# sandyz1000/face-landmark-detector

Hardware: AMD Instinct MI355X
Metric: faces/sec (whole node), 256x256 batch inference: fused preprocess + FCN-8 forward + softmax + top-4 landmark decode + similarity/alignment warp (higher is better)
Workload: dtype f32; 1 GPU; BASELINE configs[1]: batch=64/GPU 256x256x3 uint8 crops, fcn_8(68) vanilla encoder fp32, random-init weights (seed 2), decode top-4 thresh 0, align to 256x256; global_batch=64, parallelism=dp1

## Files before the change

face-landmark-detector_amd/build.py:

```python
from __future__ import annotations

import concurrent.futures
import hashlib
import os
import shutil
import subprocess
import sys

HERE = os.path.dirname(os.path.abspath(__file__))
ROOT = os.path.dirname(HERE)
CSRC = os.path.join(HERE, "csrc")
INCLUDE = os.path.join(ROOT, "include")
OBJ_DIR = os.path.join(HERE, "csrc", "build")
LIB_PATH = os.path.join(HERE, "libflm_hip.so")

SOURCES = [
    "flm_api.hip",
    "flm_pack.hip",
    "flm_enc1.hip",
    "flm_igemm.hip",
    "flm_igemm_bf16.hip",
    "flm_conv3_halo.hip",
    "flm_score1x1.hip",
    "flm_tail_bf16.hip",
    "flm_convt.hip",
    "flm_up3_wreg.hip",
    "flm_decode.hip",
    "flm_misc.hip",
    "flm_mobile.hip",
]
FLAGS = ["--offload-arch=gfx950", "-O3", "-fPIC", "-std=c++17", "-ffp-contract=off",
         "-Wall", "-Wno-unused-function", "-I", INCLUDE, "-I", CSRC]


FILE_FLAGS = {"flm_enc1.hip": ["-mllvm", "-amdgpu-mfma-vgpr-form"]}


def _hipcc() -> str:
    for c in (shutil.which("hipcc"), "/opt/rocm/bin/hipcc"):
        if c and os.path.exists(c):
            return c
    raise RuntimeError("hipcc not found: the HIP extension cannot be built")


def _stamp(paths) -> str:
    h = hashlib.sha256()
    h.update(" ".join(FLAGS).encode())
    h.update(repr(sorted(FILE_FLAGS.items())).encode())
    for p in sorted(paths):
        with open(p, "rb") as f:
            h.update(p.encode())
            h.update(f.read())
    return h.hexdigest()


def build(force: bool = False, verbose: bool = True, extra_flags=()) -> str:
    os.makedirs(OBJ_DIR, exist_ok=True)
    headers = [os.path.join(CSRC, f) for f in os.listdir(CSRC) if f.endswith(".h")] + \
              [os.path.join(INCLUDE, f) for f in os.listdir(INCLUDE) if f.endswith(".h")]
    srcs = [os.path.join(CSRC, s) for s in SOURCES]
    stamp = _stamp(srcs + headers) + " ".join(extra_flags)
    stamp_file = os.path.join(OBJ_DIR, "stamp.txt")
    if not force and os.path.exists(LIB_PATH) and os.path.exists(stamp_file) and open(stamp_file).read() == stamp:
        return LIB_PATH
    hipcc = _hipcc()

    def compile_one(src):
        obj = os.path.join(OBJ_DIR, os.path.basename(src) + ".o")
        cmd = [hipcc, *FLAGS, *FILE_FLAGS.get(os.path.basename(src), []), *extra_flags, "-c", src, "-o", obj]
        r = subprocess.run(cmd, capture_output=True, text=True)
        if r.returncode != 0:
            raise RuntimeError("hipcc failed on %s:\n%s\n%s" % (src, r.stdout, r.stderr))
        if verbose and r.stderr.strip():
            sys.stderr.write(r.stderr)
        return obj

    with concurrent.futures.ThreadPoolExecutor(max_workers=min(8, len(srcs))) as ex:
        objs = list(ex.map(compile_one, srcs))
    cmd = [hipcc, "--offload-arch=gfx950", "-shared", "-fPIC", "-o", LIB_PATH, *objs]
    r = subprocess.run(cmd, capture_output=True, text=True)
    if r.returncode != 0:
        raise RuntimeError("link failed:\n%s\n%s" % (r.stdout, r.stderr))
    with open(stamp_file, "w") as f:
        f.write(stamp)
    if verbose:
        print("built", LIB_PATH)
    return LIB_PATH


if __name__ == "__main__":
    build(force="--force" in sys.argv)
```

face-landmark-detector_amd/csrc/flm_api.hip:

```cpp
#include <cstdarg>
#include <cstdio>
#include <cstring>

#include "flm_common.h"

namespace flm {

static thread_local char g_err[512] = "";

void set_error(const char* fmt, ...) {
  va_list ap;
  va_start(ap, fmt);
  vsnprintf(g_err, sizeof(g_err), fmt, ap);
  va_end(ap);
}

int hip_fail(hipError_t e, const char* what) {
  set_error("HIP error %d (%s) at %s", (int)e, hipGetErrorString(e), what);
  return FLM_ERR_HIP;
}

struct ProfRec {
  const char* name;
  hipEvent_t a, b;
// ... 35 lines not shown
    return false;
  }
  c->enable = o->landmark_candidates != 0;
  c->sub = o->candidate_sub_phases;
  c->cap_div = o->candidate_cap_div;
  return true;
}
static int cand_sub_for(const CandOpts& c, int n_points, bool bf16) {
  if (c.sub > 0) return c.sub;
  return n_points <= 8 ? (bf16 ? 4 : 2) : (n_points <= 15 ? 6 : 8);
}
static bool landmark_candidates_enabled(const CandOpts& c, const ConvTGeom& g, int fcn32, int decode_mode, int n_points,
                                        int oh, int ow) {
  return c.enable && !fcn32 && decode_mode == FLM_DECODE_TOPN && n_points >= 1 && n_points <= 32 &&
         convt_candidates_supported(g) && (long long)oh * ow < (1 << 17);
}

struct EncNames {
  char s[kMaxEnc][8];
  EncNames() {
    for (int i = 0; i < kMaxEnc; ++i) snprintf(s[i], sizeof(s[i]), "enc%d", i + 1);
  }
};

static size_t take(size_t& cur, size_t bytes) {
  size_t o = cur;
  cur = align_up(cur + bytes, 256);
  return o;
}

Fcn8Ws fcn8_ws_layout(int n, int h, int w, int C, int dtype, int out_mode, int decode_mode, int n_points,
                      int arch, const flm_forward_opts* opts) {
  Fcn8Ws W;
  CandOpts co;
  if (!resolve_opts(opts, &co)) {
    W = Fcn8Ws();
    W.total = 0;
    return W;
  }
  const ConvTGeom g = convt_geom(C, dtype);
  const ArchSpec A = arch_spec(arch);
  const size_t es = dtype == FLM_BF16 ? 2 : 4;
  size_t cur = 0;
  int hs[kMaxEnc], wsz[kMaxEnc];
  enc_dims(A, h, w, hs, wsz);
  for (int i = 0; i < A.n_enc; ++i) W.act[i] = take(cur, es * (size_t)n * hs[i] * wsz[i] * A.enc[i].cout);
  for (int k = 0; k < 5; ++k) W.f[k] = W.act[A.f_idx[k]];
  const int h5 = h / 32, w5 = w / 32, h4 = h / 16, w4 = w / 16, h3 = h / 8, w3 = w / 8;
  W.fc6 = take(cur, es * (size_t)n * h5 * w5 * kFc);
  W.fc7 = take(cur, es * (size_t)n * h5 * w5 * kFc);
  W.score5 = take(cur, sizeof(float) * (size_t)n * h5 * w5 * g.Cp);
  W.fuse4 = take(cur, sizeof(float) * (size_t)n * h4 * w4 * g.Cp);
  W.seg = take(cur, sizeof(float) * (size_t)n * h3 * w3 * g.Cp);
  W.splitk_bytes = sizeof(float) * 8 * (size_t)n * h5 * w5 * g.Cp;
  {
    const size_t rows = (size_t)n * h5 * w5 < 256 ? (size_t)n * h5 * w5 : 256;
    const size_t fc_bytes = sizeof(float) * 8 * rows * kFc;
    if (fc_bytes > W.splitk_bytes) W.splitk_bytes = fc_bytes;
  }
  if (n <= 4) {
    const size_t enc3_bytes = sizeof(float) * 4 * (size_t)4 * (h / 4) * (w / 4) * 256;
    if (enc3_bytes > W.splitk_bytes) W.splitk_bytes = enc3_bytes;
  }
  W.splitk = take(cur, W.splitk_bytes);
  W.oh = h + (A.fcn32 ? 32 : 8);
  W.ow = w + (A.fcn32 ? 32 : 8);
  W.probs = SIZE_MAX;
  W.decode = SIZE_MAX;
  W.sub = W.tau = W.cand = W.cand_cnt = SIZE_MAX;
  W.cand_cap = 0;
  if (out_mode == FLM_OUT_LANDMARKS) {
    W.probs = take(cur, sizeof(float) * (size_t)n * W.oh * W.ow * C);
    W.decode = take(cur, decode_ws_bytes(n, W.oh, W.ow, C, decode_mode, n_points));
    if (landmark_candidates_enabled(co, g, A.fcn32, decode_mode, n_points, W.oh, W.ow)) {
      const int h3 = h / 8, w3 = w / 8;
      W.sub = take(cur, sizeof(unsigned) * (size_t)n * convt_sample_slots(g, h3, w3, cand_sub_for(co, n_points, g.bf16 != 0)) * 16 * g.MT);
      W.tau = take(cur, sizeof(float) * (size_t)n * C);
      W.cand_cap = (int)align_up((size_t)C * 64 * n_points * 4 / co.cap_div, 64);
      if (W.cand_cap < 64) W.cand_cap = 64;
      W.cand = take(cur, sizeof(unsigned long long) * (size_t)n * W.cand_cap);
      W.cand_cnt = take(cur, sizeof(unsigned) * ((size_t)n + 1));
    }
  }
  W.total = cur;
  return W;
}

static int check_fcn8_shape(int n, int h, int w, int C, int dtype) {
  if (dtype != FLM_F32 && dtype != FLM_BF16) {
    set_error("fcn8: unknown dtype %d (FLM_F32 = 0, FLM_BF16 = 1)", dtype);
    return FLM_ERR_UNSUPPORTED;
  }
  if (n <= 0 || h <= 0 || w <= 0 || (h % 32) || (w % 32)) {
    set_error("fcn8: input must be [N>0, H, W, 3] with H and W multiples of 32 (got n=%d h=%d w=%d)", n, h, w);
    return FLM_ERR_SHAPE;
  }
  if (C < 1 || C > kMaxClasses) {
    set_error("fcn8: n_classes must be in [1,%d] (got %d)", kMaxClasses, C);
    return FLM_ERR_SHAPE;
  }
  if (n > (1 << 24) || h > (1 << 15) || w > (1 << 15) || (long long)n * (h + 32) * (w + 32) * C >= (1ll << 40)) {
    set_error("fcn8: batch too large (n=%d h=%d w=%d: at most 2^40 output values per call)", n, h, w);
    return FLM_ERR_SHAPE;
  }
  return FLM_OK;
}

static int conv_layer(hipStream_t s, const char* blob, const ConvPack& c, const void* x, void* y, int n, int h,
                      int w, int relu, int pool, int posmajor, int dtype, int out_f32 = 0,
                      float* splitk_ws = nullptr, size_t splitk_bytes = 0, int stride = 1,
                      const void* res = nullptr) {
  IgemmDesc d;
  d.bf16 = dtype == FLM_BF16;
  d.out_f32 = out_f32;
  d.stride = stride;
  d.res = res;
  d.splitk_ws = splitk_ws;
  d.splitk_ws_bytes = splitk_bytes;
  d.x = x;
  d.wt = blob + c.w;
  d.scale = reinterpret_cast<const float*>(blob + c.scale);
  d.shift = reinterpret_cast<const float*>(blob + c.shift);
  d.y = y;
  d.n = n; d.h = h; d.w = w; d.cin = c.cin;
  d.cout = c.cout; d.coutpad = c.coutpad; d.ldc = c.cout;
  d.kh = c.kh; d.kw = c.kw; d.pad = c.pad;
  d.relu = relu; d.pool = pool; d.posmajor = posmajor;
  return launch_igemm(s, d);
}

}

using namespace flm;

extern "C" {

int flm_abi_version(void) { return FLM_ABI_VERSION; }

int flm_debug_query(const char* key, int arg) {
  if (key && !strcmp(key, "igemm_occupancy")) return igemm_occupancy((size_t)arg);
  return -1;
}

int flm_set_tuning(const char* key, int value) {
  if (!key) return FLM_ERR_ARG;
  if (!strcmp(key, "none")) return FLM_OK;
  if (!strcmp(key, "bf16_big_tiles")) {
    flm::igemm_bf16_big_enable(value);
    return FLM_OK;
  }
  if (!strcmp(key, "f32_two_level")) {
    flm::igemm_f32_group(value ? 0 : -1);
    return FLM_OK;
  }
  if (!strcmp(key, "bf16_mfma16")) {
    flm::igemm_bf16_big_m16(value);
    return FLM_OK;
  }
  if (!strcmp(key, "bf16_halo_mfma16")) {
    flm::conv3_halo_m16(value);
    return FLM_OK;
  }
  if (!strcmp(key, "bf16_lds_dma")) {
    flm::igemm_bf16_big_dma(value);
    return FLM_OK;
  }
  if (!strcmp(key, "landmark_candidates") || !strcmp(key, "candidate_sub_phases") || !strcmp(key, "candidate_cap_div")) {
    set_error("flm_set_tuning: '%s' changes the workspace layout and is a per-call option now: pass flm_forward_opts to "
              "flm_fcn_workspace_bytes_opts / flm_fcn_forward_opts", key);
    return FLM_ERR_ARG;
  }
  if (!strcmp(key, "up3_cand8")) {
    if (value < 0 || value > 7) {
      set_error("flm_set_tuning: up3_cand8 must be in [0,7]");
      return FLM_ERR_ARG;
    }
    flm::convt_cand8_enable(value);
    return FLM_OK;
  }
  if (!strcmp(key, "up3_cand8_rows")) {
    if (value < 0 || value > 8 || (value & (value - 1))) {
      set_error("flm_set_tuning: up3_cand8_rows must be 0, 1, 2, 4 or 8");
      return FLM_ERR_ARG;
    }
    flm::convt_cand8_rows(value);
    return FLM_OK;
  }
  if (!strcmp(key, "up3_wreg")) {
    if (value < 0 || value > 1) {
      set_error("flm_set_tuning: up3_wreg must be 0 or 1");
      return FLM_ERR_ARG;
    }
    flm::convt_wreg_enable(value);
    return FLM_OK;
  }
  if (!strcmp(key, "bf16_score1x1")) {
    flm::score1x1_enable(value);
    return FLM_OK;
  }
  if (!strcmp(key, "bf16_fused_tail")) {
    flm::tail_fused_enable(value);
    return FLM_OK;
  }
  if (!strcmp(key, "decode_lds_dma")) {
    flm::decode_dma_enable(value);
    return FLM_OK;
  }
  if (!strcmp(key, "posmajor_order")) {
    flm::igemm_posperm_enable(value);
    return FLM_OK;
  }
  if (!strcmp(key, "warp_rows")) {
    if (value != 0 && value != 1 && value != 4) {
      set_error("flm_set_tuning: warp_rows must be 0, 1 or 4");
      return FLM_ERR_ARG;
    }
    flm::warp_rows_enable(value);
    return FLM_OK;
  }
  if (!strcmp(key, "bf16_conv3_halo")) {
    flm::conv3_halo_enable(value);
    return FLM_OK;
  }
  if (!strcmp(key, "bf16_group_n")) {
    if (value < 0 || value > 32 || (value & (value - 1))) {
      set_error("flm_set_tuning: bf16_group_n must be 0 or a power of two <= 32");
      return FLM_ERR_ARG;
    }
    flm::igemm_bf16_group_n(value);
    return FLM_OK;
  }
  set_error("flm_set_tuning: unknown key '%s'", key);
  return FLM_ERR_ARG;
}

// ... 166 lines not shown
  if (!strcmp(name, "probs")) return W.probs == SIZE_MAX ? -1 : (int64_t)W.probs;
  return -1;
}

static int forward_impl(flm_stream_t stream, const void* packed_dev, const void* x_dev, int in_format, int n, int h,
                        int w, int C, int dtype, int out_mode, int decode_mode, int n_points, float thresh,
                        void* out_dev, void* workspace_dev, size_t workspace_bytes, int arch,
                        const flm_forward_opts* opts = nullptr) {
  const ArchSpec A = arch_spec(arch);
  CandOpts co;
  if (!resolve_opts(opts, &co)) return FLM_ERR_ARG;
  if (!A.valid) {
    set_error("flm_fcn_forward: unknown architecture %d", arch);
    return FLM_ERR_ARG;
  }
  const int fcn32 = A.fcn32;
  if (!packed_dev || !x_dev || !out_dev || !workspace_dev) {
    set_error("flm_fcn8_forward: null argument");
    return FLM_ERR_ARG;
  }
  int rc = check_fcn8_shape(n, h, w, C, dtype);
  if (rc) return rc;
  if (out_mode < FLM_OUT_PROBS || out_mode > FLM_OUT_LOGITS) {
    set_error("flm_fcn8_forward: unknown output mode %d", out_mode);
    return FLM_ERR_ARG;
  }
  const Fcn8Ws W = fcn8_ws_layout(n, h, w, C, dtype, out_mode, decode_mode, n_points, arch, opts);
  if (workspace_bytes < W.total) {
    set_error("flm_fcn8_forward: workspace too small (%zu < %zu)", workspace_bytes, W.total);
    return FLM_ERR_WORKSPACE;
  }
  hipStream_t s = static_cast<hipStream_t>(stream);
  const Fcn8Pack L = fcn8_pack_layout(C, dtype, arch);
  const int bf = dtype == FLM_BF16;
  const char* blob = static_cast<const char*>(packed_dev);
  char* ws = static_cast<char*>(workspace_dev);
  void* f[5];
  for (int i = 0; i < 5; ++i) f[i] = ws + W.f[i];
  void* fc6 = ws + W.fc6;
  void* fc7 = ws + W.fc7;
  float* score5 = reinterpret_cast<float*>(ws + W.score5);
  float* fuse4 = reinterpret_cast<float*>(ws + W.fuse4);
  float* seg = reinterpret_cast<float*>(ws + W.seg);

  static const EncNames enc_name_table;
  const char (*enc_names)[8] = enc_name_table.s;
  int hs[kMaxEnc], wsz[kMaxEnc];
  enc_dims(A, h, w, hs, wsz);
  {
    int h8 = hs[A.f_idx[2]], h16 = hs[A.f_idx[3]], h32 = hs[A.f_idx[4]];
    if (h8 != h / 8 || h16 != h / 16 || h32 != h / 32) {
      set_error("flm_fcn_forward: encoder grid %d/%d/%d does not match the decoder's H/8, H/16, H/32", h8, h16, h32);
      return FLM_ERR_SHAPE;
    }
  }
  for (int i = 0; i < A.n_enc; ++i) {
    const EncLayer& e = A.enc[i];
    const int src = e.src >= 0 ? e.src : i - 1;
    const void* xin = src >= 0 ? static_cast<const void*>(ws + W.act[src]) : x_dev;
    const int hi = src >= 0 ? hs[src] : h, wi = src >= 0 ? wsz[src] : w;
    void* yout = ws + W.act[i];
    const float* w0 = reinterpret_cast<const float*>(blob + (i == 0 ? L.enc1_w : L.enc[i].w));
    const float* sc0 = reinterpret_cast<const float*>(blob + (i == 0 ? L.enc1_scale : L.enc[i].scale));
    const float* sh0 = reinterpret_cast<const float*>(blob + (i == 0 ? L.enc1_shift : L.enc[i].shift));
    ProfScope ps(s, enc_names[i]);
    switch (e.kind) {
      case ENC_FIRST3:
        rc = launch_enc1(s, xin, in_format, n, hi, wi, w0, sc0, sh0, yout, bf, e.pool);
        break;
      case ENC_MB_CONV1:
        rc = launch_mb_conv1(s, xin, in_format, n, hi, wi, w0, sc0, sh0, yout, bf);
        break;
      case ENC_RN_CONV1:
        rc = launch_rn_conv1(s, xin, in_format, n, hi, wi, w0, sc0, sh0, yout, bf);
        break;
      case ENC_MAXPOOL3:
        rc = launch_maxpool3(s, xin, n, hi, wi, e.cin, yout, bf);
        break;
      case ENC_MB_DW:
        rc = launch_mb_depthwise(s, xin, n, hi, wi, e.cin, e.stride, w0, sc0, sh0, yout, bf);
        break;
      case ENC_CONV3:
        rc = conv_layer(s, blob, L.enc[i], xin, yout, n, hi, wi,  1, e.pool, 0, dtype, 0,
                        reinterpret_cast<float*>(ws + W.splitk), W.splitk_bytes);
        break;
      case ENC_MB_PW:
        if (L.enc[i].cin != e.cin) {
          int pn = n, ph = hi, pw = wi;
          if (!(pw & 1)) pw >>= 1;
          else if (!(ph & 1)) ph >>= 1;
          else if (!(pn & 1)) pn >>= 1;
          else {
            set_error("flm_fcn_forward: the paired pointwise conv needs an even number of pixels per batch");
            rc = FLM_ERR_SHAPE;
            break;
          }
          rc = conv_layer(s, blob, L.enc[i], xin, yout, pn, ph, pw,  2, 0, 0, dtype);
        } else {
          rc = conv_layer(s, blob, L.enc[i], xin, yout, n, hi, wi,  2, 0, 0, dtype);
        }
        break;
      case ENC_CONV:
        rc = conv_layer(s, blob, L.enc[i], xin, yout, n, hi, wi, e.relu, 0, 0, dtype, 0, nullptr, 0, e.stride,
                        e.res >= 0 ? ws + W.act[e.res] : nullptr);
        break;
      default:
        set_error("flm_fcn_forward: unknown encoder layer kind %d", e.kind);
        rc = FLM_ERR_ARG;
    }
    if (rc) return rc;
  }
  const int h5 = h / 32, w5 = w / 32, h4 = h / 16, w4 = w / 16, h3 = h / 8, w3 = w / 8;
  { ProfScope ps(s, "fc6");
  rc = conv_layer(s, blob, L.fc6, f[4], fc6, n, h5, w5, 1, 0,  1, dtype, 0,
                  reinterpret_cast<float*>(ws + W.splitk), W.splitk_bytes); }
  if (rc) return rc;
  { ProfScope ps(s, "fc7");
  rc = conv_layer(s, blob, L.fc7, fc6, fc7, n, h5, w5, 1, 0, 0, dtype, 0,
                  reinterpret_cast<float*>(ws + W.splitk), W.splitk_bytes); }
  if (rc) return rc;
  { ProfScope ps(s, "score5");
  rc = conv_layer(s, blob, L.score5, fc7, score5, n, h5, w5, 0, 0, 0, dtype,  1,
                  reinterpret_cast<float*>(ws + W.splitk), W.splitk_bytes); }
  if (rc) return rc;
  ConvTDesc t;
  t.g = L.g;
  t.n = n;
  if (!fcn32) {
  { ProfScope ps(s, "score4");
  rc = conv_layer(s, blob, L.score4, f[3], fuse4, n, h4, w4, 0, 0, 0, dtype, 1); }
  if (rc) return rc;
  const bool fuse_seg = bf && L.g.C == 68 && L.score3.cin == 256 && L.score3.kh == 1;
  int fused_seg = 0;
  if (!fuse_seg) {
  { ProfScope ps(s, "score3");
  rc = conv_layer(s, blob, L.score3, f[2], seg, n, h3, w3, 0, 0, 0, dtype, 1); }
  if (rc) return rc;
  }
  t.x = score5; t.wf = blob + L.up5; t.skip = fuse4; t.y = fuse4;
  t.hi = h5; t.wi = w5; t.ho = h4; t.wo = w4; t.s = 2; t.ldy = L.g.Cp; t.epilogue = 0;
  { ProfScope ps(s, "up5");
  rc = launch_convt(s, t); }
  if (rc) return rc;
  if (fuse_seg) {
    ProfScope ps(s, "seg_fused");
    fused_seg = launch_seg_fused_bf16(s, fuse4, blob + L.up4, f[2], blob + L.score3.w,
                                      reinterpret_cast<const float*>(blob + L.score3.scale),
                                      reinterpret_cast<const float*>(blob + L.score3.shift), seg, n, h4, w4, L.g.C, L.g.Cp,
                                      L.g.G, L.score3.cin, L.score3.coutpad);
    if (fused_seg < 0) return fused_seg;
  }
  if (fuse_seg && !fused_seg) {
    ProfScope ps(s, "score3");
    rc = conv_layer(s, blob, L.score3, f[2], seg, n, h3, w3, 0, 0, 0, dtype, 1);
    if (rc) return rc;
  }
  t.x = fuse4; t.wf = blob + L.up4; t.skip = seg; t.y = seg;
  t.hi = h4; t.wi = w4; t.ho = h3; t.wo = w3;
  if (!fused_seg) {
  { ProfScope ps(s, "up4");
  rc = launch_convt(s, t); }
  if (rc) return rc;
  }
  }
  t.wf = blob + L.up3; t.skip = nullptr; t.ho = W.oh; t.wo = W.ow; t.ldy = C;
  if (fcn32) { t.x = score5; t.hi = h5; t.wi = w5; t.s = 32; }
  else { t.x = seg; t.hi = h3; t.wi = w3; t.s = 8; }
// ... 199 lines not shown
```

face-landmark-detector_amd/csrc/flm_common.h:

```cpp
#pragma once

#include <hip/hip_runtime.h>
#include <stddef.h>
#include <stdint.h>

#include <atomic>
#include <mutex>

#include "flm.h"

namespace flm {

void set_error(const char* fmt, ...);
int hip_fail(hipError_t e, const char* what);

#define FLM_HIP(call)                                            \
  do {                                                           \
    hipError_t e_ = (call);                                      \
    if (e_ != hipSuccess) return ::flm::hip_fail(e_, #call);     \
  } while (0)

#define FLM_LAUNCH_CHECK(what)                                   \
  do {                                                           \
    hipError_t e_ = hipGetLastError();                           \
// ... 5 lines not shown
  std::mutex mu;
};
#define FLM_FUNC_ATTR_ONCE(flag, kernel, lds_bytes)                                                        \
  do {                                                                                                     \
    int dev_ = 0;                                                                                          \
    FLM_HIP(hipGetDevice(&dev_));                                                                          \
    const unsigned bit_ = 1u << (dev_ & 31);                                                               \
    if (!((flag).done.load(std::memory_order_acquire) & bit_)) {                                           \
      std::lock_guard<std::mutex> lock_((flag).mu);                                                        \
      if (!((flag).done.load(std::memory_order_relaxed) & bit_)) {                                         \
        FLM_HIP(hipFuncSetAttribute(reinterpret_cast<const void*>(kernel),                                 \
                                    hipFuncAttributeMaxDynamicSharedMemorySize, (int)(lds_bytes)));        \
        (flag).done.fetch_or(bit_, std::memory_order_release);                                             \
      }                                                                                                    \
    }                                                                                                      \
  } while (0)

static inline int cdiv(int a, int b) { return (a + b - 1) / b; }
static inline size_t align_up(size_t x, size_t a) { return (x + a - 1) / a * a; }

constexpr float kBnEps = 1e-3f;

constexpr int kFc = 4096;
constexpr int kMaxClasses = 96;
constexpr int kMaxEnc = 64;

enum EncKind {
  ENC_FIRST3 = 0,
  ENC_CONV3 = 1,
  ENC_MB_CONV1 = 2,
  ENC_MB_DW = 3,
  ENC_MB_PW = 4,
  ENC_RN_CONV1 = 5,
  ENC_MAXPOOL3 = 6,
  ENC_CONV = 7
};
struct EncLayer {
  int cin, cout, bn, pool;
  int kind, stride;
  int k, relu;
  int src, res;
};
struct ArchSpec {
  int n_enc;
  EncLayer enc[kMaxEnc];
  int f_idx[5];
  int fcn32;
  int valid;
};
void enc_dims(const ArchSpec& A, int h, int w, int* hs, int* ws);
inline int enc_has_params(const EncLayer& e) { return e.kind != ENC_MAXPOOL3; }
ArchSpec arch_spec(int arch);

struct ConvTGeom {
  int C;
  int Cp;
  int MT;
  int G;
  int bf16;
};
ConvTGeom convt_geom(int C, int dtype);

struct ConvPack {
  size_t w;
  size_t scale;
  size_t shift;
  int cin, cout, coutpad, kh, kw, pad;
};

struct Fcn8Pack {
  size_t enc1_w;
  size_t enc1_scale, enc1_shift;
  ConvPack enc[kMaxEnc];
  ConvPack fc6, fc7, score5, score4, score3;
  size_t up5, up4, up3;
  ConvTGeom g;
  int dtype;
  int arch;
  ArchSpec spec;
  size_t total;
};
Fcn8Pack fcn8_pack_layout(int C, int dtype, int arch = 0);

struct Fcn8Ws {
  size_t act[kMaxEnc];
  size_t f[5];
  size_t fc6, fc7, score5, fuse4, seg;
  size_t splitk;
  size_t splitk_bytes;
  size_t probs;
  size_t decode;
  size_t sub, tau, cand, cand_cnt;
  int cand_cap;
  size_t total;
  int oh, ow;
};
Fcn8Ws fcn8_ws_layout(int n, int h, int w, int C, int dtype, int out_mode, int decode_mode, int n_points,
                      int arch = 0, const flm_forward_opts* opts = nullptr);

int launch_pack_fcn(hipStream_t s, const flm_fcn_params& p, int C, const Fcn8Pack& L, char* blob);

int launch_enc1(hipStream_t s, const void* x, int in_format, int n, int h, int w, const float* w1p,
                const float* scale, const float* shift, void* f1, int out_bf16, int pool);

struct IgemmDesc {
  const void* x;
  const void* wt;
  const float* scale;
  const float* shift;
  void* y;
  int bf16;
  int out_f32;
  int n, h, w, cin;
  int cout;
  int coutpad;
  int ldc;
  int kh, kw, pad;
  int relu, pool, posmajor;
  int stride;
  const void* res;
  float* splitk_ws;
  size_t splitk_ws_bytes;
};
int launch_igemm(hipStream_t s, const IgemmDesc& d);
int igemm_occupancy(size_t lds_bytes);
void igemm_f32_group(int steps);
void igemm_bf16_big_enable(int on);
void igemm_bf16_group_n(int gn);
void igemm_bf16_big_dma(int on);
void igemm_bf16_big_m16(int on);
void conv3_halo_enable(int on);
void conv3_halo_m16(int on);
void score1x1_enable(int on);
void tail_fused_enable(int on);
void decode_dma_enable(int on);
void warp_rows_enable(int on);
void igemm_posperm_enable(int on);
int launch_seg_fused_bf16(hipStream_t s, const float* fuse4, const void* w4_packed, const void* f3, const void* w3,
                          const float* scale3, const float* shift3, float* seg, int n, int h4, int w4d, int C, int Cp,
                          int G, int cin3, int coutpad3);

struct ConvTDesc {
  const float* x;
  const void* wf;
  const float* skip;
  void* y;
  int n, hi, wi;
  int ho, wo;
  int s;
  int ldy;
  int epilogue;
  ConvTGeom g;
  int sub = 0;
  const float* tau = nullptr;
  unsigned long long* cand = nullptr;
  unsigned* cand_cnt = nullptr;
  int cand_cap = 0;
  const unsigned* gate = nullptr;
  void* scratch = nullptr;
  size_t scratch_bytes = 0;
};
int launch_convt(hipStream_t s, const ConvTDesc& d);
int convt_candidates_supported(const ConvTGeom& g);
__host__ __device__ inline int convt_share_layout(const ConvTGeom& g, int s) {
  return g.C == 68 && (g.bf16 ? g.G == 9 : g.G == 17) && (s % 4) == 0;
}
int convt_sample_slots(const ConvTGeom& g, int hi, int wi, int sub);
void convt_cand8_enable(int mask);
void convt_cand8_rows(int rpw);
void convt_wreg_enable(int on);
int launch_cand_tau(hipStream_t s, const unsigned* wave_max, int n, int slots, int ld, int l, int n_points, float* tau);

int launch_mb_conv1(hipStream_t s, const void* x, int in_format, int n, int h, int w, const float* wgt,
                    const float* scale, const float* shift, void* y, int bf16);
int launch_mb_depthwise(hipStream_t s, const void* x, int n, int h, int w, int c, int stride, const float* wgt,
                        const float* scale, const float* shift, void* y, int bf16);
int launch_rn_conv1(hipStream_t s, const void* x, int in_format, int n, int h, int w, const float* wgt,
                    const float* scale, const float* shift, void* y, int bf16);
int launch_maxpool3(hipStream_t s, const void* x, int n, int h, int w, int c, void* y, int bf16);

size_t decode_ws_bytes(int n, int h, int w, int l, int mode, int n_points);
int launch_decode(hipStream_t s, const float* hm, int n, int h, int w, int l, int ld, int mode, int n_points,
                  float thresh, double* out, void* ws, size_t ws_bytes, float* tau_out = nullptr,
                  const unsigned* gate = nullptr);
size_t decode_sweep_ws_bytes(int n, int h, int w, int l, const int* modes, int n_modes);
int launch_decode_sweep(hipStream_t s, const float* hm, int n, int h, int w, int l, const int* modes, int n_modes,
                        float thresh, double* out, void* ws, size_t ws_bytes);
int launch_gaussian_heatmaps(hipStream_t s, const double* kp, int n, int l, int h, int w, double two_sigma_sq,
                             float* out);
int launch_cand_merge(hipStream_t s, const unsigned long long* cand, unsigned* cand_cnt, int n, int w, int l,
                      int n_points, float thresh, int cap, double* out);

int launch_preprocess(hipStream_t s, const uint8_t* img, int n, int h, int w, int norm, float* out);
int launch_similarity(hipStream_t s, const double* lm, const double* tmpl, int n, int k, double sx, double sy, float* m);
int launch_warp(hipStream_t s, const void* src, int src_is_u8, int n, int hs, int ws, const float* m, float* dst,
                int hd, int wd);
int launch_crop_resize(hipStream_t s, const uint8_t* frame, int fh, int fw, const int32_t* boxes, int k,
                       uint8_t* out, int oh, int ow, const int32_t* frame_idx = nullptr, size_t frame_stride = 0,
                       int nframes = 0);

__device__ __forceinline__ int xcd_remap(int b, int nblk) {
  const int q = nblk >> 3, r = nblk & 7;
  const int xcd = b & 7, loc = b >> 3;
  const int base = (xcd < r) ? xcd * (q + 1) : r * (q + 1) + (xcd - r) * q;
  return base + loc;
}

// ... 2 lines not shown
```

face-landmark-detector_amd/csrc/flm_igemm.hip:

```cpp
#include <vector>

#include "flm_igemm_args.h"

#ifndef FLM_IGEMM_VAR
#define FLM_IGEMM_VAR 0
#endif

namespace flm {

typedef float f32x16 __attribute__((ext_vector_type(16)));
typedef __bf16 bf16x8 __attribute__((ext_vector_type(8)));

constexpr int BM = 128, BN = 128, BK = 32;
constexpr int TILE_F = BM * BK;

__device__ __forceinline__ int swz(int row, int chunk) { return row * BK + ((chunk ^ ((row >> 1) & 7)) << 2); }

__device__ __forceinline__ float f4c(const float4& v, int i) { return i == 0 ? v.x : (i == 1 ? v.y : (i == 2 ? v.z : v.w)); }

template <bool BF, int IDX>
__device__ __forceinline__ void mfma_slot(const float4& a0, const float4& a1, const float4& b0, const float4& b1,
                                          f32x16& c00, f32x16& c01, f32x16& c10, f32x16& c11) {
  if constexpr (BF) {
    const float4& av = (IDX >> 1) ? a1 : a0;
// ... 578 lines not shown
  for (size_t i = (size_t)blockIdx.x * blockDim.x + threadIdx.x; i < total; i += (size_t)gridDim.x * blockDim.x) {
    const int c = (int)(i % ldc);
    if (c >= cout) continue;
    float v = 0.f;
    for (int s = 0; s < ksplit; ++s) v += part[(size_t)s * total + i];
    v = fmaf(v, scale[c], shift[c]);
    if (relu) v = fmaxf(v, 0.f);
    if (out_bf16) reinterpret_cast<unsigned short*>(y)[i] = f2bf(v);
    else reinterpret_cast<float*>(y)[i] = v;
  }
}

__global__ void splitk_reduce_pool_kernel(const float* __restrict__ part, const float* __restrict__ scale,
                                          const float* __restrict__ shift, void* __restrict__ y, int M, int ldc, int cout,
                                          int ksplit, int relu, float relu_max, int out_bf16) {
  const size_t total = (size_t)(M >> 2) * ldc, plane = (size_t)M * ldc;
  for (size_t i = (size_t)blockIdx.x * blockDim.x + threadIdx.x; i < total; i += (size_t)gridDim.x * blockDim.x) {
    const int c = (int)(i % ldc);
    if (c >= cout) continue;
    const size_t q = i / ldc;
    float best = -3.402823466e38f;
#pragma unroll
    for (int e = 0; e < 4; ++e) {
      float v = 0.f;
      for (int s = 0; s < ksplit; ++s) v += part[(size_t)s * plane + (4 * q + e) * ldc + c];
      v = fmaf(v, scale[c], shift[c]);
      if (relu) v = fminf(fmaxf(v, 0.f), relu_max);
      best = fmaxf(best, v);
    }
    if (out_bf16) reinterpret_cast<unsigned short*>(y)[i] = f2bf(best);
    else reinterpret_cast<float*>(y)[i] = best;
  }
}

int igemm_occupancy(size_t lds_bytes) {
  int nb = -1;
  if (hipOccupancyMaxActiveBlocksPerMultiprocessor(&nb, reinterpret_cast<const void*>(&igemm_kernel<false, 0, true>), 256,
                                                   lds_bytes) != hipSuccess)
    return -1;
  return nb;
}

template <bool BF, bool TWO = false>
static int dispatch(hipStream_t s, const IgemmDesc& d, const IgemmArgs& a) {
  if (d.pool) return d.relu ? launch_t<BF, 1, true, TWO>(s, a) : launch_t<BF, 1, false, TWO>(s, a);
  if (d.posmajor) return d.relu ? launch_t<BF, 2, true, TWO>(s, a) : launch_t<BF, 2, false, TWO>(s, a);
  return d.relu ? launch_t<BF, 0, true, TWO>(s, a) : launch_t<BF, 0, false, TWO>(s, a);
}

static std::atomic<int> g_f32_group{0};
void igemm_f32_group(int steps) { g_f32_group = steps; }

int launch_igemm(hipStream_t s, const IgemmDesc& d) {
  const int es = d.bf16 ? 2 : 4;
  const int bke = 128 / es;
  if (d.cin % bke != 0 || d.coutpad % BN != 0 || d.cout > d.coutpad || d.kh * d.kw > 64) {
    set_error("igemm: unsupported shape cin=%d coutpad=%d cout=%d k=%dx%d (%s)", d.cin, d.coutpad, d.cout, d.kh, d.kw,
              d.bf16 ? "bf16" : "fp32");
    return FLM_ERR_SHAPE;
  }
  if (d.pool && ((d.h & 1) || (d.w & 1))) {
    set_error("igemm: pooled layer needs even h,w (got %dx%d)", d.h, d.w);
    return FLM_ERR_SHAPE;
  }
  const int stride = d.stride > 0 ? d.stride : 1;
  const int ho = (d.h + 2 * d.pad - d.kh) / stride + 1, wo = (d.w + 2 * d.pad - d.kw) / stride + 1;
  if ((stride != 1 || d.res) && (d.pool || d.posmajor)) {
    set_error("igemm: stride / residual are only built for the row-major pixel order");
    return FLM_ERR_UNSUPPORTED;
  }
  if (stride == 1 && (ho != d.h || wo != d.w)) {
    set_error("igemm: stride-1 layers must be 'same' (k=%dx%d pad=%d)", d.kh, d.kw, d.pad);
    return FLM_ERR_SHAPE;
  }
  const long long M = (long long)d.n * ho * wo;
  if (M <= 0 || M > (1ll << 30)) {
    set_error("igemm: pixel count %lld out of range", M);
    return FLM_ERR_SHAPE;
  }
  if ((long long)d.n * d.h * d.w * d.cin * es >= (1ll << 32) || (long long)d.coutpad * d.kh * d.kw * d.cin >= (1ll << 31)) {
    set_error("igemm: tensor exceeds the 32-bit offset range (split the batch)");
    return FLM_ERR_SHAPE;
  }
  IgemmArgs a;
  a.x = d.x; a.wt = d.wt; a.scale = d.scale; a.shift = d.shift; a.y = d.y;
  a.out_f32 = d.bf16 ? d.out_f32 : 1;
  a.relu_max = d.relu == 2 ? 6.0f : 3.402823466e38f;
  a.n = d.n; a.h = d.h; a.w = d.w; a.cin = d.cin; a.cout = d.cout; a.ldc = d.ldc;
  a.ho = ho; a.wo = wo; a.stride = stride; a.res = d.res;
  a.kh = d.kh; a.kw = d.kw; a.pad = d.pad;
  a.M = (int)M;
  a.K = d.kh * d.kw * d.cin;
  a.mtiles = cdiv(a.M, BM);
  a.cpt = d.cin / bke;
  a.kw_magic = (65536 + d.kw - 1) / d.kw;
  a.ksplit = 1;
  a.gm = a.gn = 1;
  a.grp_magic = 0;
  a.posperm_on = 0;
  for (int k = 0; k < 8; ++k) a.posperm[k] = 0ull;
  a.part = nullptr;
  const int tiles = cdiv(a.M, BM) * cdiv(d.cout, BN);
  const int faces = d.n > 0 ? d.n : 1;
  const bool few_faces = d.kh * d.kw > 1 && d.cout < 1024 && faces <= 4 && tiles <= 64 * faces;
  const bool narrow_1x1 = !d.bf16 && d.kh * d.kw == 1 && d.cin / bke >= 32 && d.cout <= BN;
  const int tile_cap = narrow_1x1 ? 0x7fffffff : ((d.cout >= 1024 || few_faces) ? 256 : 64);
  if (d.splitk_ws && !d.res && stride == 1 && tiles <= tile_cap && (!d.pool || (a.M & 3) == 0) &&
      (d.kh * d.kw == 1 ? a.cpt >= 32 : (a.cpt >= 4 && (d.cout >= 1024 || tiles <= 16 * faces || few_faces))) &&
      (d.relu != 2 || d.pool)) {
    int ks = (tiles <= 64 || narrow_1x1) ? 8 : (tiles <= 128 ? 4 : 2);
    if (few_faces && tiles > 16 * faces) ks = 8;
    int per = d.kh * d.kw == 1 ? 8 : 1;
    if (d.kh * d.kw == 1 && tiles <= 8) {
      ks = 32;
      per = 4;
    }
    if (d.kh * d.kw > 1) {
      if (ks > d.kh * d.kw * a.cpt / 8) ks = d.kh * d.kw * a.cpt / 8;
    } else if (ks > a.cpt / per) {
      ks = a.cpt / per;
    }
    const size_t part_rows = few_faces ? (size_t)(a.M / faces) * 4 : (size_t)a.M;
    if (ks > 1 && (size_t)ks * part_rows * d.ldc * sizeof(float) <= d.splitk_ws_bytes) {
      a.ksplit = ks;
      a.part = d.splitk_ws;
    }
  }
  a.ntiles = cdiv(d.cout, BN);
  if (d.bf16) {
    const int sk = launch_score1x1_bf16(s, a, d.relu, d.pool, d.posmajor, d.coutpad);
    if (sk < 0) return sk;
    if (sk == 1) return FLM_OK;
    const int halo = launch_conv3_halo_bf16(s, a, d.relu, d.pool, d.posmajor);
    if (halo < 0) return halo;
    if (halo == 1) return FLM_OK;
    const int big = launch_igemm_bf16_big(s, a, d.relu, d.pool, d.posmajor, d.coutpad);
    if (big < 0) return big;
    if (big == 1) return FLM_OK;
  }
  int rc;
  const int f32_knob = g_f32_group.load(std::memory_order_relaxed);
  if (d.bf16) {
    rc = dispatch<true>(s, d, a);
  } else if (f32_knob < 0) {
    rc = dispatch<false>(s, d, a);
  } else {
    const int dense = d.kh * d.kw * a.cpt;
    if (dense >= 8192) {
      set_error("igemm: %d k-steps per output exceed the group divider's range", dense);
      return FLM_ERR_SHAPE;
    }
    int grp = 2;
    while ((grp + 1) * (grp + 1) <= dense) ++grp;
    a.grp_magic = (65536 + grp - 1) / grp;
    const long long face_in = (long long)d.h * d.w * d.cin * 4,
                    face_out = (long long)(d.pool ? (ho / 2) * (wo / 2) : ho * wo) * d.ldc * 4;
    const long long lim = (1ll << 31) - (1ll << 22);
    if (face_in >= lim) {
      set_error("igemm: one face exceeds the 2 GiB buffer range of the fp32 kernel");
      return FLM_ERR_SHAPE;
    }
    const int max_faces = (int)(lim / face_in);
    if (d.n <= max_faces) {
      rc = dispatch<false, true>(s, d, a);
    } else {
      if (a.ksplit > 1) {
// ... 33 lines not shown
```

Before: 7691 faces/s.

## Add Winograd F(2x2,3x3) fp32 conv path for pooled encoder layers

```diff
diff --git a/face-landmark-detector_amd/build.py b/face-landmark-detector_amd/build.py
--- a/face-landmark-detector_amd/build.py
+++ b/face-landmark-detector_amd/build.py
@@ -19,6 +19,7 @@
     "flm_pack.hip",
     "flm_enc1.hip",
     "flm_igemm.hip",
+    "flm_wino.hip",
     "flm_igemm_bf16.hip",
     "flm_conv3_halo.hip",
     "flm_score1x1.hip",
diff --git a/face-landmark-detector_amd/csrc/flm_api.hip b/face-landmark-detector_amd/csrc/flm_api.hip
--- a/face-landmark-detector_amd/csrc/flm_api.hip
+++ b/face-landmark-detector_amd/csrc/flm_api.hip
@@ -141,6 +141,11 @@
       W.cand_cnt = take(cur, sizeof(unsigned) * ((size_t)n + 1));
     }
   }
+  for (int i = 0; i < 5; ++i) W.wino[i] = SIZE_MAX;
+  if (dtype == FLM_F32 && (arch == FLM_ARCH_FCN8 || arch == FLM_ARCH_FCN32) && n >= kWinoMinFaces)
+    for (int i = 1; i < 5 && i < A.n_enc; ++i)
+      if ((kWinoLayers >> i) & 1)
+        W.wino[i] = take(cur, sizeof(float) * 16 * (size_t)A.enc[i].cin * align_up(A.enc[i].cout, 128));
   W.total = cur;
   return W;
 }
@@ -168,7 +173,7 @@
 static int conv_layer(hipStream_t s, const char* blob, const ConvPack& c, const void* x, void* y, int n, int h,
                       int w, int relu, int pool, int posmajor, int dtype, int out_f32 = 0,
                       float* splitk_ws = nullptr, size_t splitk_bytes = 0, int stride = 1,
-                      const void* res = nullptr) {
+                      const void* res = nullptr, float* wino = nullptr) {
   IgemmDesc d;
   d.bf16 = dtype == FLM_BF16;
   d.out_f32 = out_f32;
@@ -185,6 +190,7 @@
   d.cout = c.cout; d.coutpad = c.coutpad; d.ldc = c.cout;
   d.kh = c.kh; d.kw = c.kw; d.pad = c.pad;
   d.relu = relu; d.pool = pool; d.posmajor = posmajor;
+  d.wino = wino;
   return launch_igemm(s, d);
 }
 
@@ -210,6 +216,10 @@
   }
   if (!strcmp(key, "f32_two_level")) {
     flm::igemm_f32_group(value ? 0 : -1);
+    return FLM_OK;
+  }
+  if (!strcmp(key, "f32_winograd")) {
+    flm::igemm_f32_winograd(value);
     return FLM_OK;
   }
   if (!strcmp(key, "bf16_mfma16")) {
@@ -542,7 +552,8 @@
         break;
       case ENC_CONV3:
         rc = conv_layer(s, blob, L.enc[i], xin, yout, n, hi, wi,  1, e.pool, 0, dtype, 0,
-                        reinterpret_cast<float*>(ws + W.splitk), W.splitk_bytes);
+                        reinterpret_cast<float*>(ws + W.splitk), W.splitk_bytes, 1, nullptr,
+                        i < 5 && W.wino[i] != SIZE_MAX ? reinterpret_cast<float*>(ws + W.wino[i]) : nullptr);
         break;
       case ENC_MB_PW:
         if (L.enc[i].cin != e.cin) {
diff --git a/face-landmark-detector_amd/csrc/flm_common.h b/face-landmark-detector_amd/csrc/flm_common.h
--- a/face-landmark-detector_amd/csrc/flm_common.h
+++ b/face-landmark-detector_amd/csrc/flm_common.h
@@ -111,8 +111,12 @@
 };
 Fcn8Pack fcn8_pack_layout(int C, int dtype, int arch = 0);
 
+constexpr unsigned kWinoLayers = 0x1eu;
+constexpr int kWinoMinFaces = 17;
+
 struct Fcn8Ws {
   size_t act[kMaxEnc];
+  size_t wino[5];
   size_t f[5];
   size_t fc6, fc7, score5, fuse4, seg;
   size_t splitk;
@@ -150,8 +154,12 @@
   const void* res;
   float* splitk_ws;
   size_t splitk_ws_bytes;
+  float* wino = nullptr;
 };
 int launch_igemm(hipStream_t s, const IgemmDesc& d);
+int launch_wino(hipStream_t s, const IgemmDesc& d);
+void igemm_f32_winograd(int on);
+int igemm_f32_winograd_enabled();
 int igemm_occupancy(size_t lds_bytes);
 void igemm_f32_group(int steps);
 void igemm_bf16_big_enable(int on);
diff --git a/face-landmark-detector_amd/csrc/flm_igemm.hip b/face-landmark-detector_amd/csrc/flm_igemm.hip
--- a/face-landmark-detector_amd/csrc/flm_igemm.hip
+++ b/face-landmark-detector_amd/csrc/flm_igemm.hip
@@ -684,6 +684,9 @@
     set_error("igemm: tensor exceeds the 32-bit offset range (split the batch)");
     return FLM_ERR_SHAPE;
   }
+  if (!d.bf16 && d.wino && d.n > 16 && g_f32_group.load(std::memory_order_relaxed) >= 0 && igemm_f32_winograd_enabled() &&
+      d.pool && d.kh == 3 && d.kw == 3 && d.pad == 1 && stride == 1 && !d.res && d.cin % 16 == 0 && d.coutpad % 64 == 0)
+    return launch_wino(s, d);
   IgemmArgs a;
   a.x = d.x; a.wt = d.wt; a.scale = d.scale; a.shift = d.shift; a.y = d.y;
   a.out_f32 = d.bf16 ? d.out_f32 : 1;
diff --git a/face-landmark-detector_amd/csrc/flm_wino.hip b/face-landmark-detector_amd/csrc/flm_wino.hip
--- /dev/null
+++ b/face-landmark-detector_amd/csrc/flm_wino.hip
@@ -0,0 +1,305 @@
+#include "flm_igemm_args.h"
+
+namespace flm {
+
+namespace {
+
+typedef float f32x16 __attribute__((ext_vector_type(16)));
+
+constexpr int kTY = 4, kTX = 8;
+constexpr int kPH = 2 * kTY + 2, kPW = 2 * kTX + 2;
+constexpr int kUStep = 16 * 2 * 64 * 4;
+constexpr int kVStep = 16 * 2 * 32 * 4;
+constexpr int kPStep = 8 * 64 * 4;
+constexpr int kUSlots = 3, kPSlots = 3;
+constexpr int kLdsFloats = kUSlots * kUStep + 2 * kVStep + kPSlots * kPStep;
+
+struct WinoArgs {
+  const float* x;
+  const float* u;
+  const float* scale;
+  const float* shift;
+  float* y;
+  float relu_max;
+  int n, h, w, cin, cout, ldc;
+  int th, tw;
+  int bty, btx;
+  int npanel;
+  int upanels;
+};
+
+__device__ __forceinline__ float4 f4add(float4 a, float4 b) { return make_float4(a.x + b.x, a.y + b.y, a.z + b.z, a.w + b.w); }
+__device__ __forceinline__ float4 f4sub(float4 a, float4 b) { return make_float4(a.x - b.x, a.y - b.y, a.z - b.z, a.w - b.w); }
+__device__ __forceinline__ float4 f4sel(bool c, float4 a, float4 b) {
+  return make_float4(c ? a.x : b.x, c ? a.y : b.y, c ? a.z : b.z, c ? a.w : b.w);
+}
+__device__ __forceinline__ float f4c(const float4& v, int i) { return i == 0 ? v.x : (i == 1 ? v.y : (i == 2 ? v.z : v.w)); }
+
+__device__ __forceinline__ void lds_barrier() { asm volatile("s_waitcnt lgkmcnt(0)\n\ts_barrier" ::: "memory"); }
+
+template <bool RELU>
+__global__ __launch_bounds__(512, 1) void wino_kernel(WinoArgs a) {
+  extern __shared__ __attribute__((aligned(16))) float sm[];
+  float* Ub = sm;
+  float* Vb = sm + kUSlots * kUStep;
+  float* Pb = Vb + 2 * kVStep;
+
+  const int tid = threadIdx.x, lane = tid & 63, wave = tid >> 6;
+  const int L = xcd_remap(blockIdx.x, gridDim.x);
+  const int per_panel = a.n * a.bty * a.btx;
+  const int panel = L / per_panel;
+  int rest = L - panel * per_panel;
+  const int bx = rest % a.btx;
+  rest /= a.btx;
+  const int by = rest % a.bty;
+  const int face = rest / a.bty;
+  const int ty0 = by * kTY, tx0 = bx * kTX;
+  const int S = a.cin >> 3;
+
+  typedef __attribute__((address_space(3))) char lds_char;
+  const int wave_u = __builtin_amdgcn_readfirstlane(wave);
+  const unsigned lds0 = (unsigned)(size_t)((lds_char*)sm);
+  const unsigned lds_u = lds0 + wave_u * 4096, lds_p = lds0 + (kUSlots * kUStep + 2 * kVStep) * 4 + wave_u * 1024;
+  const dma_srd usrd = dma_make_srd(a.u + (size_t)panel * kUStep);
+  const dma_srd xsrd = dma_make_srd(a.x + (size_t)face * a.h * a.w * a.cin);
+  const unsigned uvoff = (unsigned)(wave * 4096 + lane * 16);
+  const int ustep_bytes = a.upanels * kUStep * 4;
+  unsigned pvoff;
+  {
+    const int q = tid, pp = q >> 1, pr = pp / kPW, pc = pp - pr * kPW;
+    const int iy = 2 * ty0 - 1 + pr, ix = 2 * tx0 - 1 + pc;
+    const bool ok = q < kPH * kPW * 2 && iy >= 0 && iy < a.h && ix >= 0 && ix < a.w;
+    pvoff = ok ? (unsigned)(((iy * a.w + ix) * a.cin + 4 * (q & 1)) * 4) : kOobOffset;
+  }
+
+  const int tt = tid & 31, tq = (tid >> 5) & 1, ti = (tid >> 6) & 3, tjh = tid >> 8;
+  const int ra = ti == 0 ? 0 : (ti == 2 ? 2 : 1), rb = ti == 0 ? 2 : (ti == 1 ? 2 : (ti == 2 ? 1 : 3));
+  const bool radd = ti == 1;
+  const int pa = ((2 * (tt >> 3) + ra) * kPW + 2 * (tt & 7) + tjh) * 8 + 4 * tq;
+  const int pb = ((2 * (tt >> 3) + rb) * kPW + 2 * (tt & 7) + tjh) * 8 + 4 * tq;
+  const int xo = 4 * ti + 2 * tjh;
+  const int vo0 = ((xo * 2 + tq) * 32 + tt) * 4, vo1 = (((xo + 1) * 2 + tq) * 32 + tt) * 4;
+
+  const int lr = lane & 31, lh = lane >> 5;
+  const int xw = 2 * wave;
+  const int wave_s = __builtin_amdgcn_readfirstlane(wave);
+  const int va = ((xw * 2 + lh) * 32 + lr) * 4;
+  const int ua = ((xw * 2 + lh) * 64 + lr) * 4;
+
+#define WINO_DMA(S_, USLOT, PS_, PSLOT)                                                              \
+  {                                                                                                  \
+    const int us_ = (S_) < S ? (S_) : S - 1, ps_ = (PS_) < S ? (PS_) : S - 1;                        \
+    const unsigned mu_ = lds_u + (USLOT) * (kUStep * 4);                                             \
+    dma_load16(usrd, mu_, uvoff, us_ * ustep_bytes);                                                 \
+    dma_load16(usrd, mu_ + 1024, uvoff, us_ * ustep_bytes + 1024);                                   \
+    dma_load16(usrd, mu_ + 2048, uvoff, us_ * ustep_bytes + 2048);                                   \
+    dma_load16(usrd, mu_ + 3072, uvoff, us_ * ustep_bytes + 3072);                                   \
+    dma_load16(xsrd, lds_p + (PSLOT) * (kPStep * 4), pvoff, ps_ * 32);                               \
+  }
+#define WINO_TRANSFORM(PSLOT, VBUF)                                                                \
+  {                                                                                          \
+    const float* p_ = Pb + (PSLOT) * kPStep;                                                 \
+    const float4 a0 = *reinterpret_cast<const float4*>(p_ + pa);                             \
+    const float4 a1 = *reinterpret_cast<const float4*>(p_ + pa + 8);                         \
+    const float4 a2 = *reinterpret_cast<const float4*>(p_ + pa + 16);                        \
+    const float4 b0 = *reinterpret_cast<const float4*>(p_ + pb);                             \
+    const float4 b1 = *reinterpret_cast<const float4*>(p_ + pb + 8);                         \
+    const float4 b2 = *reinterpret_cast<const float4*>(p_ + pb + 16);                        \
+    const float4 r0 = f4sel(radd, f4add(a0, b0), f4sub(a0, b0));                             \
+    const float4 r1 = f4sel(radd, f4add(a1, b1), f4sub(a1, b1));                             \
+    const float4 r2 = f4sel(radd, f4add(a2, b2), f4sub(a2, b2));                             \
+     \
+    const float4 e_ = f4sub(r0, r2);                                                         \
+    const float4 f_ = f4sel(tjh, f4sub(r1, r0), f4add(r1, r2));                              \
+    float* v_ = Vb + (VBUF) * kVStep;                                                        \
+    *reinterpret_cast<float4*>(v_ + vo0) = f4sel(tjh, f_, e_);                               \
+    *reinterpret_cast<float4*>(v_ + vo1) = f4sel(tjh, e_, f_);                               \
+  }
+
+  f32x16 acc00, acc01, acc10, acc11, sum00, sum01, sum10, sum11, zero16;
+#pragma unroll
+  for (int r = 0; r < 16; ++r)
+    acc00[r] = acc01[r] = acc10[r] = acc11[r] = sum00[r] = sum01[r] = sum10[r] = sum11[r] = zero16[r] = 0.f;
+
+#define WINO_MFMA(BUF, USLOT, FIRST)                                                                        \
+  {                                                                                                  \
+    const float* v_ = Vb + (BUF) * kVStep + va;                                                      \
+    const float* u_ = Ub + (USLOT) * kUStep + ua;                                                    \
+    const float4 A0 = *reinterpret_cast<const float4*>(v_);                                          \
+    const float4 A1 = *reinterpret_cast<const float4*>(v_ + 256);                                    \
+    const float4 B00 = *reinterpret_cast<const float4*>(u_);                                         \
+    const float4 B01 = *reinterpret_cast<const float4*>(u_ + 128);                                   \
+    const float4 B10 = *reinterpret_cast<const float4*>(u_ + 512);                                   \
+    const float4 B11 = *reinterpret_cast<const float4*>(u_ + 640);                                   \
+    _Pragma("unroll") for (int e = 0; e < 4; ++e) {                                                  \
+      const bool z_ = (FIRST) && e == 0;                                                             \
+      acc00 = __builtin_amdgcn_mfma_f32_32x32x2f32(f4c(A0, e), f4c(B00, e), z_ ? zero16 : acc00, 0, 0, 0); \
+      acc01 = __builtin_amdgcn_mfma_f32_32x32x2f32(f4c(A0, e), f4c(B01, e), z_ ? zero16 : acc01, 0, 0, 0); \
+      acc10 = __builtin_amdgcn_mfma_f32_32x32x2f32(f4c(A1, e), f4c(B10, e), z_ ? zero16 : acc10, 0, 0, 0); \
+      acc11 = __builtin_amdgcn_mfma_f32_32x32x2f32(f4c(A1, e), f4c(B11, e), z_ ? zero16 : acc11, 0, 0, 0); \
+    }                                                                                                \
+  }
+
+#define WINO_STEP(S_, BUF, FIRST)                                                  \
+  {                                                                                \
+    const int uc_ = uslot, un_ = uslot == 2 ? 0 : uslot + 1, uf_ = un_ == 2 ? 0 : un_ + 1;  \
+    WINO_DMA((S_) + 2, uf_, (S_) + 3, uc_)                                         \
+    if (wave_s < 4) {                                                              \
+      WINO_MFMA(BUF, uc_, FIRST)                                                   \
+      WINO_TRANSFORM(un_, (BUF) ^ 1)                                               \
+    } else {                                                                       \
+      WINO_TRANSFORM(un_, (BUF) ^ 1)                                               \
+      WINO_MFMA(BUF, uc_, FIRST)                                                   \
+    }                                                                              \
+    asm volatile("s_waitcnt vmcnt(5) lgkmcnt(0)\n\ts_barrier" ::: "memory");     \
+    uslot = un_;                                                                   \
+  }
+
+  WINO_DMA(0, 0, 0, 0)
+  WINO_DMA(1, 1, 1, 1)
+  dma_load16(xsrd, lds_p + 2 * (kPStep * 4), pvoff, (S > 2 ? 2 : S - 1) * 32);
+  asm volatile("s_waitcnt vmcnt(0)\n\ts_barrier" ::: "memory");
+  WINO_TRANSFORM(0, 0)
+  lds_barrier();
+
+  int uslot = 0;
+  for (int s = 0; s < S; s += 2) {
+    WINO_STEP(s, 0, true)
+    WINO_STEP(s + 1, 1, false)
+    sum00 += acc00;
+    sum01 += acc01;
+    sum10 += acc10;
+    sum11 += acc11;
+  }
+  asm volatile("s_waitcnt vmcnt(0) lgkmcnt(0)\n\ts_barrier" ::: "memory");
+#undef WINO_DMA
+#undef WINO_TRANSFORM
+#undef WINO_MFMA
+#undef WINO_STEP
+
+  float* mx = sm;
+#pragma unroll
+  for (int j = 0; j < 2; ++j) {
+    if (j) lds_barrier();
+    const f32x16& s0 = j ? sum01 : sum00;
+    const f32x16& s1 = j ? sum11 : sum10;
+#pragma unroll
+    for (int r = 0; r < 16; ++r) {
+      const int t = (r & 3) + 8 * (r >> 2) + 4 * lh;
+      mx[(xw * 32 + t) * 32 + lr] = s0[r];
+      mx[((xw + 1) * 32 + t) * 32 + lr] = s1[r];
+    }
+    lds_barrier();
+    const int cl = tid & 31;
+    const int col = panel * 64 + 32 * j + cl;
+    const float sc = a.scale[col], sh = a.shift[col];
+#pragma unroll
+    for (int k = 0; k < 2; ++k) {
+      const int t = (tid >> 5) + 16 * k;
+      double m[16];
+#pragma unroll
+      for (int xi = 0; xi < 16; ++xi) m[xi] = (double)mx[(xi * 32 + t) * 32 + cl];
+      double q0[4], q1[4];
+#pragma unroll
+      for (int b = 0; b < 4; ++b) {
+        q0[b] = (m[b] + m[4 + b]) + m[8 + b];
+        q1[b] = (m[4 + b] - m[8 + b]) - m[12 + b];
+      }
+      const float y00 = (float)((q0[0] + q0[1]) + q0[2]), y01 = (float)((q0[1] - q0[2]) - q0[3]);
+      const float y10 = (float)((q1[0] + q1[1]) + q1[2]), y11 = (float)((q1[1] - q1[2]) - q1[3]);
+      float v = -3.402823466e38f;
+      const float yy[4] = {y00, y01, y10, y11};
+#pragma unroll
+      for (int e = 0; e < 4; ++e) {
+        float u = fmaf(yy[e], sc, sh);
+        if (RELU) u = fminf(fmaxf(u, 0.f), a.relu_max);
+        v = fmaxf(v, u);
+      }
+      const int ty = ty0 + (t >> 3), tx = tx0 + (t & 7);
+      if (col < a.cout && ty < a.th && tx < a.tw) a.y[(((size_t)face * a.th + ty) * a.tw + tx) * a.ldc + col] = v;
+    }
+  }
+}
+
+__global__ void wino_u_kernel(const float* __restrict__ wt, float* __restrict__ u, int cin, int coutpad) {
+  const int P = coutpad / 64, K = 9 * cin;
+  const int total = cin * coutpad;
+  for (int i = blockIdx.x * blockDim.x + threadIdx.x; i < total; i += gridDim.x * blockDim.x) {
+    const int e = i & 3, col = (i >> 2) & 63, h = (i >> 8) & 1, rest = i >> 9;
+    const int p = rest % P, st = rest / P;
+    const int c = 8 * st + 4 * h + e, o = 64 * p + col;
+    const float* g = wt + (size_t)o * K + c;
+    double t[4][3];
+#pragma unroll
+    for (int kx = 0; kx < 3; ++kx) {
+      const double g0 = g[(0 * 3 + kx) * cin], g1 = g[(1 * 3 + kx) * cin], g2 = g[(2 * 3 + kx) * cin];
+      t[0][kx] = g0;
+      t[1][kx] = 0.5 * (g0 + g1 + g2);
+      t[2][kx] = 0.5 * (g0 - g1 + g2);
+      t[3][kx] = g2;
+    }
+    float* d = u + (((size_t)st * P + p) * 16 * 2 + h) * 256 + col * 4 + e;
+#pragma unroll
+    for (int a = 0; a < 4; ++a) {
+      d[(4 * a + 0) * 512] = (float)t[a][0];
+      d[(4 * a + 1) * 512] = (float)(0.5 * (t[a][0] + t[a][1] + t[a][2]));
+      d[(4 * a + 2) * 512] = (float)(0.5 * (t[a][0] - t[a][1] + t[a][2]));
+      d[(4 * a + 3) * 512] = (float)t[a][2];
+    }
+  }
+}
+
+std::atomic<int> g_wino{1};
+
+}
+
+void igemm_f32_winograd(int on) { g_wino.store(on ? 1 : 0, std::memory_order_relaxed); }
+int igemm_f32_winograd_enabled() { return g_wino.load(std::memory_order_relaxed); }
+
+int launch_wino(hipStream_t s, const IgemmDesc& d) {
+  if (!d.wino || d.bf16 || !d.pool || d.kh != 3 || d.kw != 3 || d.pad != 1 || (d.stride > 1) || d.res || (d.cin % 16) ||
+      (d.coutpad % 64) || d.cout > d.coutpad || (d.h & 1) || (d.w & 1)) {
+    set_error("wino: unsupported layer (cin=%d cout=%d k=%dx%d pad=%d pool=%d)", d.cin, d.cout, d.kh, d.kw, d.pad, d.pool);
+    return FLM_ERR_SHAPE;
+  }
+  WinoArgs a;
+  a.x = reinterpret_cast<const float*>(d.x);
+  a.u = d.wino;
+  a.scale = d.scale;
+  a.shift = d.shift;
+  a.y = reinterpret_cast<float*>(d.y);
+  a.relu_max = d.relu == 2 ? 6.0f : 3.402823466e38f;
+  a.n = d.n; a.h = d.h; a.w = d.w; a.cin = d.cin; a.cout = d.cout; a.ldc = d.ldc;
+  a.th = d.h / 2;
+  a.tw = d.w / 2;
+  a.bty = cdiv(a.th, kTY);
+  a.btx = cdiv(a.tw, kTX);
+  a.npanel = cdiv(d.cout, 64);
+  a.upanels = d.coutpad / 64;
+  const long long blocks = (long long)d.n * a.bty * a.btx * a.npanel;
+  if (blocks <= 0 || blocks >= (1ll << 31)) {
+    set_error("wino: %lld workgroups out of range", blocks);
+    return FLM_ERR_SHAPE;
+  }
+  if ((long long)d.h * d.w * d.cin * 4 >= (1ll << 31) - (1ll << 22) || 64ll * d.cin * d.coutpad >= (1ll << 31)) {
+    set_error("wino: face or filter exceeds the 2 GiB buffer range (h=%d w=%d cin=%d coutpad=%d)", d.h, d.w, d.cin, d.coutpad);
+    return FLM_ERR_SHAPE;
+  }
+  wino_u_kernel<<<cdiv(d.cin * d.coutpad, 256) < 2048 ? cdiv(d.cin * d.coutpad, 256) : 2048, 256, 0, s>>>(
+      reinterpret_cast<const float*>(d.wt), d.wino, d.cin, d.coutpad);
+  FLM_LAUNCH_CHECK("wino_u_kernel");
+  const size_t lds = sizeof(float) * kLdsFloats;
+  if (d.relu) {
+    static FuncAttrOnce attr;
+    FLM_FUNC_ATTR_ONCE(attr, (&wino_kernel<true>), lds);
+    wino_kernel<true><<<(unsigned)blocks, 512, lds, s>>>(a);
+  } else {
+    static FuncAttrOnce attr;
+    FLM_FUNC_ATTR_ONCE(attr, (&wino_kernel<false>), lds);
+    wino_kernel<false><<<(unsigned)blocks, 512, lds, s>>>(a);
+  }
+  FLM_LAUNCH_CHECK("wino_kernel");
+  return FLM_OK;
+}
+
+}
```

Measured after the change: 8232 faces/s (median of 6 runs). 1.07x the previous value.
